# wsntxxn/AudioCaption

Measured on AMD Instinct MI355X. Metric: clips/sec (10 s @ 32 kHz) encode+greedy-decode, Cnn14_Rnn-Trm, higher is better.
Workload: dtype bf16x3

## Files before the change

### audiocaption_amd/_lib.py

```python
import ctypes
import os

import torch

_HERE = os.path.dirname(os.path.abspath(__file__))
LIB_PATH = os.environ.get("AUDIOCAPTION_HIP_LIB") or os.path.join(_HERE, "libaudiocaption_hip.so")

AC_MAX_LAYERS = 8
AC_ENS_MAX = 8
ABI_VERSION = 2

c_float_p = ctypes.c_void_p
c_int_p = ctypes.c_void_p


class AcTrmLayer(ctypes.Structure):
    _fields_ = [(n, ctypes.c_void_p) for n in (
        "sa_in_w", "sa_in_b", "sa_out_w", "sa_out_b", "ca_in_w", "ca_in_b", "ca_out_w", "ca_out_b",
        "l1_w", "l1_b", "l2_w", "l2_b", "n1_w", "n1_b", "n2_w", "n2_b", "n3_w", "n3_b")]


class AcTrmWeights(ctypes.Structure):
    _fields_ = [(n, ctypes.c_int32) for n in (
        "d_model", "nhead", "nlayers", "dim_ff", "vocab", "max_pos", "attn_emb_dim", "reserved")] + [
        (n, ctypes.c_void_p) for n in ("emb", "pe", "cls_w", "proj_w", "proj_b", "proj_ln_w", "proj_ln_b", "step_pk")] + [
        ("layer", AcTrmLayer * AC_MAX_LAYERS)]


class AcTrmKeyword(ctypes.Structure):
    _fields_ = [("kwp", ctypes.c_void_p), ("ln_w", ctypes.c_void_p), ("ln_b", ctypes.c_void_p), ("row_div", ctypes.c_int32)]


class AcLogitRules(ctypes.Structure):
    _fields_ = [("repetition_penalty", ctypes.c_float), ("no_repeat_ngram", ctypes.c_int32), ("min_length", ctypes.c_int32),
                ("end_idx", ctypes.c_int32), ("n_bad", ctypes.c_int32), ("bad_words", ctypes.c_void_p)]


class AcBahWeights(ctypes.Structure):
    _fields_ = [(n, ctypes.c_int32) for n in (
        "emb_dim", "d_model", "attn_size", "attn_emb_dim", "fc_emb_dim", "vocab", "n_tags", "variant")] + [
        (n, ctypes.c_void_p) for n in ("emb", "temb", "w_ih", "w_hh", "b_ih", "b_hh", "attn_w", "attn_b", "attn_v",
                                       "fc_w", "fc_b", "ctx_w", "ctx_b", "cls_w", "cls_b")]


class AcBahGrads(ctypes.Structure):
    _fields_ = [(n, ctypes.c_void_p) for n in ("emb", "temb", "w_ih", "w_hh", "b_ih", "b_hh", "attn_w", "attn_b", "attn_v",
                                               "fc_w", "fc_b", "ctx_w", "ctx_b", "cls_w", "cls_b")]


_I, _L, _F, _P = ctypes.c_int, ctypes.c_long, ctypes.c_float, ctypes.c_void_p
_U64 = ctypes.c_ulonglong
_WP = ctypes.POINTER(AcTrmWeights)
_BP = ctypes.c_void_p

SIGNATURES = {
    "ac_abi_version": (_I, []),
    "ac_logmel": (_I, [_P, _I, _I, _I, _I, _P, _P, _P, _P, _P, _P, _P, _P, _I, _L, _L, _L, _P]),
    "ac_conv3x3_bn_relu": (_I, [_P, _P, _P, _P, _P, _I, _I, _I, _I, _I, _I, _I, _I, _P]),
    "ac_conv3x3_bn_relu_winograd": (_I, [_P, _P, _P, _P, _P, _I, _I, _I, _I, _I, _I, _I, _I, _P]),
    "ac_conv3x3_bn_relu_bf16x3": (_I, [_P, _P, _P, _P, _P, _I, _I, _I, _I, _I, _I, _I, _I, _P]),
    "ac_conv3x3_bn_relu_bf16x3_gw": (_I, [_P, _P, _P, _P, _P, _I, _I, _I, _I, _I, _I, _I, _I, _P]),
    "ac_conv3x3_bn_relu_wino1d": (_I, [_P, _P, _P, _P, _P, _I, _I, _I, _I, _I, _I, _I, _I, _P, _I, _I, _P]),
    "ac_conv3x3_bn_relu_wino1d_drop": (_I, [_P, _P, _P, _P, _P, _I, _I, _I, _I, _I, _I, _I, _I, _F, _U64, _P, _P]),
    "ac_conv3x3_wino1d_splitk_floats": (_L, [_I, _I, _I, _I, _I]),
    "ac_conv3x3_bn_relu_wino1d_splitk": (_I, [_P, _P, _P, _P, _P, _I, _I, _I, _I, _I, _I, _I, _I, _P, _I, _I, _P, _L, _P]),
    "ac_conv3x3_bn_relu_wino43": (_I, [_P, _P, _P, _P, _P, _I, _I, _I, _I, _I, _I, _I, _I, _I, _P, _I, _I, _P]),
    "ac_conv3x3_bn_relu_wino43_drop": (_I, [_P, _P, _P, _P, _P, _I, _I, _I, _I, _I, _I, _I, _I, _F, _U64, _P, _P]),
    "ac_conv3x3_wino43_workgroups": (_L, [_I, _I, _I, _I]),
    "ac_conv3x3_block1_wino43": (_I, [_P, _P, _P, _P, _P, _P, _P, _P, _I, _I, _I, _P, _I, _I, _F, _U64, _P, _P]),
    "ac_conv3x3_block1_wino43_mfma": (_I, [_P, _P, _P, _P, _P, _P, _P, _P, _I, _I, _I, _P, _I, _I, _F, _U64, _P, _P]),
    "ac_conv3x3_block1_conv2_wino43": (_I, [_P, _P, _P, _P, _P, _I, _I, _I, _P]),
    "ac_conv3x3_bn_relu_f16x2_gw": (_I, [_P, _P, _P, _P, _P, _I, _I, _I, _I, _I, _I, _I, _I, _I, _P, _P]),
    "ac_conv3x3_block1_f16x2": (_I, [_P, _P, _P, _P, _P, _P, _P, _P, _I, _I, _I, _I, _P, _P]),
    "ac_linear_bf16x3": (_I, [_P, _P, _P, _P, _P, _I, _I, _I, _I, _P]),
    "ac_conv3x3_first": (_I, [_P, _P, _P, _P, _P, _I, _I, _I, _I, _P]),
    "ac_conv3x3_first_f16": (_I, [_P, _P, _P, _P, _P, _I, _I, _I, _I, _P, _P]),
    "ac_linear": (_I, [_P, _P, _P, _P, _I, _I, _I, _L, _L, _L, _I, _P]),
    "ac_gru_pack_whh": (_I, [_P, _P, _I, _P]),
    "ac_gru_layer": (_I, [_P, _P, _P, _P, _P, _I, _I, _I, _P]),
    "ac_gru_split_workspace_bytes": (_L, [_I]),
    "ac_gru_layer_split": (_I, [_P, _P, _P, _P, _P, _P, _P, _I, _I, _I, _P]),
    "ac_mean_with_lens": (_I, [_P, _P, _P, _I, _I, _I, _I, _P]),
    "ac_add_layernorm": (_I, [_P, _P, _P, _P, _P, _I, _I, _L, _L, _L, _P]),
    "ac_trm_memory": (_I, [_WP, _P, _I, _I, _P, _P, _P]),
    "ac_trm_step_pack_floats": (_L, [_WP]),
    "ac_trm_pack_step_weights": (_I, [_WP, _P, _P]),
    "ac_dec_wide_packed_floats": (_L, [_I, _I]),
    "ac_dec_wide_pack": (_I, [_P, _L, _I, _I, _P, _P]),
    "ac_dec_wide_gemm": (_I, [_I, _P, _L, _P, _L, _P, _P, _P, _L, _I, _P, _P, _F, _P, _L, _P, _P, _P, _L, _I, _I, _I, _I, _I, _I, _P]),
    "ac_trm_workspace_floats": (_L, [_WP, _I, _I]),
    "ac_trm_greedy": (_I, [_WP, _P, _P, _I, _I, _I, _I, _I, _I, _P, _P, _P, _P, _P, _P, _P]),
    "ac_trm_greedy_segments": (_I, [_WP, _P, _P, _I, _I, _I, _I, _I, _I, _I, _P, _P, _P, _P, _P, _P, _P]),
    "ac_sample_rows": (_I, [_P, _L, _I, _I, _I, _I, _F, _F, _P, _I, _P, _P, _P]),
    "ac_trm_sample": (_I, [_WP, _P, _P, _I, _I, _I, _I, _I, _I, _P, _P, _P, _P, _P, _P, _I, _I, _F, _F, _P, _P]),
    "ac_trm_sample_multi": (_I, [_WP, _P, _P, _I, _I, _I, _I, _I, _I, _I, _P, _P, _P, _P, _P, _P, _I, _I, _F, _F, _P, _P]),
    "ac_conv3x3_skinny_workspace_floats": (_L, [_I, _I, _I, _I, _I]),
    "ac_conv3x3_bn_relu_skinny": (_I, [_P, _P, _P, _P, _P, _I, _I, _I, _I, _I, _I, _I, _P, _L, _F, _U64, _P, _P]),
    "ac_trm_cluster_pack_floats": (_L, [_WP]),
    "ac_trm_cluster_pack": (_I, [_WP, _P, _P]),
    "ac_trm_cluster_workspace_bytes": (_L, [_I]),
    "ac_trm_greedy_cluster": (_I, [_WP, _P, _P, _P, _I, _I, _I, _I, _I, _I, _P, _P, _P, _P, _P, _P, _I, _P]),
    "ac_trm_forward_tokens": (_I, [_WP, _P, _P, _I, _I, _P, _P, _I, _P, _P, _P, _P]),
    "ac_trm_beam_step": (_I, [_WP, _P, _P, _I, _I, _I, _I, _I, _F, _P, _P, _P, _P, _P, _P, _P]),
    "ac_trm_beam_update": (_I, [_P, _P, _P, _P, _P, _P, _P, _P, _P, _P, _P, _P, _I, _I, _I, _I, _I, _I, _I, _I, _P]),
    "ac_trm_beam_reorder": (_I, [_WP, _I, _I, _I, _P, _P, _P]),
    "ac_trm_beam_update_all": (_I, [_P, _P, _P, _P, _P, _P, _P, _P, _P, _P, _P, _P, _I, _I, _I, _I, _I, _I, _I, _I, _P]),
    "ac_trm_kw_greedy_segments": (_I, [_WP, _P, _P, _P, _I, _I, _I, _I, _I, _I, _I, _P, _P, _P, _P, _P, _P, _P]),
    "ac_trm_kw_sample": (_I, [_WP, _P, _P, _P, _I, _I, _I, _I, _I, _I, _P, _P, _P, _P, _P, _P, _I, _I, _F, _F, _P, _P]),
    "ac_trm_kw_forward_tokens": (_I, [_WP, _P, _P, _P, _I, _I, _P, _P, _I, _P, _P, _P, _P]),
    "ac_trm_kw_beam_step": (_I, [_WP, _P, _P, _P, _I, _I, _I, _I, _I, _F, _P, _P, _P, _P, _P, _P, _P]),
    "ac_trm_kw_embed_qkv": (_I, [_WP, _P, _I, _I, _I, _P, _L, _P, _P, _P]),
    "ac_trm_step_logits": (_I, [_WP, _P, _P, _I, _I, _I, _I, _I, _P, _P, _I, _P, _L, _P, _L, _P, _P]),
    "ac_ens_greedy_pick": (_I, [_P, _I, _L, _I, _I, _I, _I, _I, _I, _P, _P, _P, _P, _P, _P, _P]),
    "ac_ens_sample_pick": (_I, [_P, _I, _L, _I, _I, _I, _I, _F, _F, _P, _I, _I, _I, _I, _P, _P, _P, _P, _P, _P, _P, _P]),
    "ac_ens_beam_step_select": (_I, [_P, _I, _L, _I, _I, _I, _I, _F, _P, _P, _P, _P, _P]),
    "ac_logit_rules_apply": (_I, [_P, _L, _P, _L, _I, _I, _P, _L, _I, _P, _P]),
    "ac_trm_search_rules": (_I, [_WP, _P, _P, _I, _I, _I, _I, _I, _I, _I, _P, _P, _P, _P, _P, _P, _I, _I, _F, _F, _P, _P, _P, _L,
                                 _P]),
    "ac_trm_beam_step_rules": (_I, [_WP, _P, _P, _I, _I, _I, _I, _I, _F, _P, _P, _P, _P, _P, _P, _P, _P, _P]),
    "ac_bah_workspace_floats": (_L, [_BP, _I, _I, _I, _I]),
    "ac_bah_memory": (_I, [_BP, _P, _P, _I, _I, _I, _I, _P, _P]),
    "ac_bah_memory_cond": (_I, [_BP, _P, _P, _I, _I, _I, _I, _P, _P]),
    "ac_bah_step_logits": (_I, [_BP, _P, _P, _I, _I, _I, _I, _I, _P, _P, _L, _P, _P, _P, _L, _P, _L, _P, _L, _L, _P, _P]),
    "ac_bah_greedy": (_I, [_BP, _P, _P, _P, _I, _I, _I, _I, _I, _I, _P, _P, _P, _P, _P, _P, _P, _P, _P]),
    "ac_bah_sample": (_I, [_BP, _P, _P, _P, _I, _I, _I, _I, _I, _I, _P, _P, _P, _P, _P, _P, _P, _P, _I, _I, _F, _F, _P, _P]),
    "ac_bah_beam_gather": (_I, [_P, _P, _P, _P, _P, _P, _P, _I, _I, _I, _I, _I, _I, _P]),
    "ac_bah_train_workspace_floats": (_L, [_BP, _I, _I, _I]),
    "ac_bah_train_forward": (_I, [_BP, _P, _P, _P, _P, _L, _P, _P, _I, _I, _I, _I, _F, _U64, _P, _P, _P, _P, _P, _P, _P, _P,
                                  _P]),
    "ac_bah_train_rollout": (_I, [_BP, _P, _P, _P, _P, _I, _I, _I, _I, _I, _F, _P, _P, _L, _F, _U64, _P, _P, _P, _P, _P, _P, _P,
                                  _P, _P, _P]),
    "ac_bah_train_backward": (_I, [_BP, _P, _P, _P, _P, _P, _I, _I, _I, _F, _U64, _P, _P, _P, _P, _P]),
    "ac_bah_train_forward_cond": (_I, [_BP, _P, _P, _P, _P, _L, _P, _I, _I, _I, _I, _F, _U64, _P, _P, _P, _P, _P, _P, _P, _P,
                                       _P]),
# ... 162 lines not shown
```

### audiocaption_amd/build.py

```python
import hashlib
import os
import shutil
import subprocess
import sys

HERE = os.path.dirname(os.path.abspath(__file__))
CSRC = os.path.join(HERE, "csrc")
LIB = os.path.join(HERE, "libaudiocaption_hip.so")
STAMP = LIB + ".stamp"
SOURCES = ["logmel.hip", "conv3x3.hip", "conv3x3_winograd.hip", "conv3x3_wino1d.hip", "conv3x3_wino43.hip", "conv3x3_block1_w4.hip", "conv3x3_skinny.hip", "gemm.hip", "gru.hip", "decoder.hip", "decoder_wide.hip", "decoder_cluster.hip", "sample.hip", "ensemble.hip", "logit_rules.hip", "attn_gru.hip", "attn_gru_train.hip", "spec_loss.hip", "sed.hip", "train.hip", "scst.hip", "kd.hip", "enc_kd.hip", "cider.hip", "capmetrics.hip", "diversity.hip", "effnet.hip", "effnet_fused.hip", "pw_gemm.hip", "ingest.hip", "probe.hip"]
FLAGS = ["--offload-arch=gfx950", "-O3", "-std=c++17", "-fPIC", "-Wall",
         "-Wno-unused-function", "-Wno-unused-result"]
NO_PACKED_F32 = ["-Xclang", "-target-feature", "-Xclang", "-packed-fp32-ops"]
EXTRA_FLAGS = {"sed.hip": ["-ffp-contract=off"], "enc_kd.hip": ["-ffp-contract=off"]}

def _hipcc():
    for c in (os.environ.get("HIPCC"), "/opt/rocm/bin/hipcc", shutil.which("hipcc")):
        if c and os.path.exists(c):
            return c
    raise RuntimeError("hipcc not found (expected /opt/rocm/bin/hipcc)")


def _digest():
    h = hashlib.sha256()
    for root in (CSRC, os.path.join(os.path.dirname(HERE), "include")):
        for name in sorted(os.listdir(root)):
            with open(os.path.join(root, name), "rb") as f:
                h.update(name.encode())
                h.update(f.read())
    h.update(" ".join(FLAGS).encode())
    h.update(repr((NO_PACKED_F32, sorted(EXTRA_FLAGS.items()))).encode())
    return h.hexdigest()


def _up_to_date(digest):
    if os.path.exists(LIB) and os.path.exists(STAMP):
        with open(STAMP) as f:
            return f.read().strip() == digest
    return False


def build(force=False, verbose=False):
    import fcntl
    digest = _digest()
    if not force and _up_to_date(digest):
        return LIB
    os.makedirs(os.path.join(HERE, "build"), exist_ok=True)
    with open(os.path.join(HERE, "build", ".lock"), "w") as lock:
        fcntl.flock(lock, fcntl.LOCK_EX)
        try:
            if not force and _up_to_date(digest):
                return LIB
            return _compile(digest, verbose)
        finally:
            fcntl.flock(lock, fcntl.LOCK_UN)


def _compile(digest, verbose):
    hipcc = _hipcc()
    objs = []
    procs = []
    os.makedirs(os.path.join(HERE, "build"), exist_ok=True)
    for src in SOURCES:
# ... 26 lines not shown
```

### audiocaption_amd/csrc/gru.hip

```cpp
#include "ac_common.h"

namespace {

struct GruParams {
  const float* gx;
  const float* whhT;
  const float* bhh;
  const int* lens;
  float* out;
  int B, T;
};

constexpr int H = 256;

__device__ __forceinline__ float sigmoidf_(float x) { return 1.0f / (1.0f + expf(-x)); }

constexpr int GRU_KREG = 96, GRU_KLDS = 48;
__global__ __launch_bounds__(768) void gru_layer_kernel(GruParams p) {
  __shared__ __attribute__((aligned(16))) float sh[H];
  __shared__ float sg[3 * H];
  extern __shared__ __attribute__((aligned(16))) float swl[];
  const int n = threadIdx.x;
  const int b = blockIdx.x >> 1, dir = blockIdx.x & 1;
  int len = p.lens[b];
// ... 171 lines not shown
  if (c >= C) return;
  const int len = lens[b];
  float s = 0.f;
  for (int t = 0; t < len && t < T; ++t) s += x[((size_t)b * T + t) * C + c];
  out[(size_t)b * C + c] = s / (float)len;
}

__global__ void maxmean_lens_kernel(const float* x, const int* lens, float* out, int T, int C) {
  const int b = blockIdx.x, c = blockIdx.y * blockDim.x + threadIdx.x;
  if (c >= C) return;
  const int len = lens[b];
  float s = 0.f, m = -INFINITY;
  for (int t = 0; t < len && t < T; ++t) {
    const float v = x[((size_t)b * T + t) * C + c];
    s += v;
    m = fmaxf(m, v);
  }
  out[(size_t)b * C + c] = m + s / (float)len;
}

__global__ void gru_pack_whh_kernel(const float* whh, float* packed, int total) {
  const int i = blockIdx.x * blockDim.x + threadIdx.x;
  if (i >= total) return;
  const int kk = i & 3, n = (i >> 2) % (3 * H), k4 = ((i >> 2) / (3 * H)) % (H / 4), d = i / (3 * H * H);
  packed[i] = whh[((size_t)d * 3 * H + n) * H + k4 * 4 + kk];
}

}

extern "C" int ac_gru_pack_whh(const float* whh, float* packed, int hidden, void* stream) {
  if (!whh || !packed || hidden != H) return AC_ERR_ARG;
  const int total = 2 * 3 * H * H;
  hipLaunchKernelGGL(gru_pack_whh_kernel, dim3((total + 255) / 256), dim3(256), 0, (hipStream_t)stream, whh, packed, total);
  return ac_check_launch();
}

extern "C" int ac_gru_layer(const float* gx, const float* whhT, const float* bhh, const int* lens, float* out,
                            int B, int T, int hidden, void* stream) {
  if (!gx || !whhT || !bhh || !lens || !out || B <= 0 || T <= 0 || hidden != H) return AC_ERR_ARG;
  GruParams p;
  p.gx = gx; p.whhT = whhT; p.bhh = bhh; p.lens = lens; p.out = out; p.B = B; p.T = T;
  const size_t lds = (size_t)GRU_KLDS * 3 * H * sizeof(float);
  static AcLdsAttr lds_attr;
  if (ac_allow_lds((const void*)gru_layer_kernel, (int)lds, &lds_attr) != AC_OK) return AC_ERR_LAUNCH;
  hipLaunchKernelGGL(gru_layer_kernel, dim3(2 * B), dim3(768), lds, (hipStream_t)stream, p);
  return ac_check_launch();
}

extern "C" long ac_gru_split_workspace_bytes(int B) {
  if (B <= 0) return AC_ERR_ARG;
  return 128 + (long)B * 2 * GQ * 2 * HQ * 8;
}

extern "C" int ac_gru_layer_split(const float* gx, const float* whh, const float* bhh, const int* lens, float* out,
                                  float* save, void* workspace, int B, int T, int hidden, void* stream) {
  if (!gx || !whh || !bhh || !lens || !out || !workspace || B <= 0 || T <= 0 || hidden != H) return AC_ERR_ARG;
  const size_t gran = (size_t)B * 2 * GQ * 2 * HQ * 8;
  GruSplitParams p;
  p.gx = gx; p.whh = whh; p.bhh = bhh; p.lens = lens; p.out = out; p.save = save; p.B = B; p.T = T;
  p.error = (unsigned*)workspace;
  p.ticket = (unsigned*)((char*)workspace + 64);
  p.xch = (unsigned long long*)((char*)workspace + 128);
  {
    const unsigned words = (unsigned)((64 + gran) / 8);
    hipLaunchKernelGGL(gru_split_reset_kernel, dim3((words + 255) / 256), dim3(256), 0, (hipStream_t)stream,
                       (unsigned long long*)((char*)workspace + 64), words);
  }
  hipLaunchKernelGGL(gru_layer_split_kernel, dim3(2 * GQ * B), dim3(256), 0, (hipStream_t)stream, p);
  return ac_check_launch();
}

extern "C" int ac_mean_with_lens(const float* x, const int* lens, float* out, int B, int T, int C, int add_max,
                                 void* stream) {
  if (!x || !lens || !out || B <= 0 || T <= 0 || C <= 0) return AC_ERR_ARG;
  if (add_max)
    hipLaunchKernelGGL(maxmean_lens_kernel, dim3(B, (C + 255) / 256), dim3(256), 0, (hipStream_t)stream, x, lens, out, T, C);
  else
    hipLaunchKernelGGL(mean_lens_kernel, dim3(B, (C + 255) / 256), dim3(256), 0, (hipStream_t)stream, x, lens, out, T, C);
  return ac_check_launch();
}
```

### audiocaption_amd/kernels.py

```python
import contextlib
import ctypes
import os

import torch

from . import _lib
from ._lib import check, f32c, ptr, stream


def upload(t, device, dtype=None):
    t = torch.as_tensor(t)
    if t.is_cuda:
        return t.to(device=device, dtype=dtype)
    if dtype is not None:
        t = t.to(dtype)
    pin = torch.empty(t.shape, dtype=t.dtype, pin_memory=True)
    pin.copy_(t)
    return pin.to(device, non_blocking=True)


def _dev(t):
    if not t.is_cuda:
        raise _lib.HipLibraryError("the HIP path needs tensors on a ROCm device; there is no CPU fallback")
    return t
# ... 261 lines not shown

    return torch.stack([lay(hi), lay(lo)], dim=3).contiguous()


def pack_conv_weight_winograd(w):
    cout, cin = w.shape[0], w.shape[1]

    def g_times(t, dim):
        t0, t1, t2 = t.select(dim, 0), t.select(dim, 1), t.select(dim, 2)
        return torch.stack([t0, 0.5 * (t0 + t1 + t2), 0.5 * (t0 - t1 + t2), t2], dim=dim)

    out = torch.empty(cin // 32, 4, 4, cout, 32, device=w.device, dtype=torch.float32)
    step = max(1, (1 << 22) // (cin * 16))
    for o0 in range(0, cout, step):
        u = g_times(g_times(w[o0:o0 + step].double(), 2), 3)
        u = u.permute(1, 3, 2, 0).reshape(cin // 32, 32, 4, 4, -1).permute(0, 2, 3, 4, 1)
        out[:, :, :, o0:o0 + step] = u.float()
    return out


def pack_conv_weight(w):
    cout, cin = w.shape[0], w.shape[1]
    return (w.permute(1, 2, 3, 0).reshape(cin // 32, 32, 9, cout).permute(0, 2, 3, 1).contiguous())


def fold_bn(bn_weight, bn_bias, mean, var, eps):
    scale = bn_weight / torch.sqrt(var + eps)
    return scale.contiguous(), (bn_bias - mean * scale).contiguous()


LINEAR_ALGO = os.environ.get("AUDIOCAPTION_LINEAR_ALGO", "bf16x3")
_LINEAR_PACKS = {}


def pack_linear_weight_bf16x3_frag(w):
    n, k = w.shape
    return pack_conv_weight_bf16x3_frag(w.reshape(n, k, 1, 1))


def _linear_pack(w):
    import weakref
    hit = _LINEAR_PACKS.get(id(w))
    if hit is not None and hit[0]() is w and hit[1] == w._version and hit[2] == _lib.param_generation():
        return hit[3:]
    for k in [k for k, v in _LINEAR_PACKS.items() if v[0]() is None]:
        del _LINEAR_PACKS[k]
    with torch.no_grad():
        pack = (pack_linear_weight_bf16x3_frag(w.detach().float()), torch.ones(w.shape[0], device=w.device),
                torch.zeros(w.shape[0], device=w.device))
    _LINEAR_PACKS[id(w)] = (weakref.ref(w), w._version, _lib.param_generation()) + pack
    return pack


def linear(x, w, b=None, relu=False, out=None):
    lib = _lib.load()
    M, K = x.shape
    N = w.shape[0]
    if out is None:
        out = torch.empty(M, N, device=x.device, dtype=torch.float32)
    if (LINEAR_ALGO == "bf16x3" and N * K >= 1536 * 512 and K % 32 == 0 and N % 64 == 0 and x.stride(0) == K
            and out.stride(0) == N and w.is_contiguous()):
        wfrag, ones, zeros = _linear_pack(w)
        check(lib.ac_linear_bf16x3(ptr(x), ptr(wfrag), ptr(ones), ptr(b if b is not None else zeros), ptr(out), M, N, K,
                                   1 if relu else 0, stream()), "ac_linear_bf16x3")
        return out
    check(lib.ac_linear(ptr(x), ptr(w), ptr(b), ptr(out), M, N, K, x.stride(0), w.stride(0), out.stride(0),
                        1 if relu else 0, stream()), "ac_linear")
    return out


def gru_pack_whh(whh, hidden):
    lib = _lib.load()
    whh = f32c(_dev(whh))
    out = torch.empty_like(whh)
    check(lib.ac_gru_pack_whh(ptr(whh), ptr(out), hidden, stream()), "ac_gru_pack_whh")
    return out


def gru_layer(gx, whhT, bhh, lens_i32, B, T, hidden):
    lib = _lib.load()
    out = torch.empty(B, T, 2 * hidden, device=gx.device, dtype=torch.float32)
    check(lib.ac_gru_layer(ptr(gx), ptr(whhT), ptr(bhh), ptr(lens_i32), ptr(out), B, T, hidden, stream()),
          "ac_gru_layer")
    return out


def gru_layer_split(gx, whh, bhh, lens_i32, B, T, hidden, workspace=None):
    lib = _lib.load()
    need = lib.ac_gru_split_workspace_bytes(B)
    if workspace is None or workspace.numel() * 8 < need or workspace.device != gx.device:
        workspace = torch.zeros((need + 7) // 8, device=gx.device, dtype=torch.int64)
    out = torch.empty(B, T, 2 * hidden, device=gx.device, dtype=torch.float32)
    check(lib.ac_gru_layer_split(ptr(gx), ptr(whh), ptr(bhh), ptr(lens_i32), ptr(out), None, ptr(workspace), B, T, hidden,
                                 stream()), "ac_gru_layer_split")
    return out, workspace


def gru_split_error(workspace, B):
    return workspace.view(torch.int32)[:1]


def mean_with_lens(x, lens_i32, add_max=False):
    lib = _lib.load()
    B, T, C = x.shape
    out = torch.empty(B, C, device=x.device, dtype=torch.float32)
    check(lib.ac_mean_with_lens(ptr(x), ptr(lens_i32), ptr(out), B, T, C, 1 if add_max else 0, stream()),
          "ac_mean_with_lens")
    return out


def add_layernorm(x, y, w, b, out=None):
    lib = _lib.load()
    rows, d = x.shape
    if out is None:
        out = torch.empty(rows, d, device=x.device, dtype=torch.float32)
    check(lib.ac_add_layernorm(ptr(x), ptr(y), ptr(w), ptr(b), ptr(out), rows, d, x.stride(0),
                               y.stride(0) if y is not None else 0, out.stride(0), stream()), "ac_add_layernorm")
    return out


def dropout_(x, n, p, seed, seed_dev=None):
    lib = _lib.load()
    check(lib.ac_dropout(ptr(x), ptr(x), n, float(p), int(seed), seed_dev, 0, stream()), "ac_dropout")
    return x


def rows_mean_w(x, out, B, Hp, H, W, C):
    lib = _lib.load()
    check(lib.ac_rows_mean_w(ptr(x), ptr(out), B, Hp, H, W, C, stream()), "ac_rows_mean_w")
    return out


def specaug_(x, stripes, fill, B, rows_per_clip, T, n_time=2, n_freq=2):
    lib = _lib.load()
    check(lib.ac_specaug(ptr(x), ptr(stripes), ptr(fill), B, rows_per_clip, T, 64, n_time, n_freq, stream()), "ac_specaug")
    return x


def specaug_stripes(seed, B, T, F=64, time_width=64, time_num=2, freq_width=8, freq_num=2):
    import numpy as np
    rng = np.random.default_rng(int(seed) & 0xFFFFFFFFFFFFFFFF)
    out = np.zeros((B, time_num + freq_num, 2), dtype=np.int32)
    for b in range(B):
        for k in range(time_num):
            d = int(rng.integers(0, time_width))
            out[b, k] = (int(rng.integers(0, T - d)), d)
    for b in range(B):
# ... 43 lines not shown
```

### audiocaption_amd/rnn_encoder.py

```python
import os

import torch
import torch.nn as nn

from . import kernels as K


class RnnEncoder(nn.Module):

    def __init__(self, spec_dim, fc_feat_dim, attn_feat_dim, pooling="mean", **kwargs):
        super().__init__()
        self.spec_dim, self.fc_feat_dim, self.attn_feat_dim = spec_dim, fc_feat_dim, attn_feat_dim
        self.pooling = pooling
        self.hidden_size = kwargs.get("hidden_size", 512)
        self.bidirectional = kwargs.get("bidirectional", False)
        self.num_layers = kwargs.get("num_layers", 1)
        self.dropout = kwargs.get("dropout", 0.2)
        self.rnn_type = kwargs.get("rnn_type", "GRU")
        self.in_bn = kwargs.get("in_bn", False)
        self.embed_dim = self.hidden_size * (self.bidirectional + 1)
        if self.rnn_type != "GRU" or not self.bidirectional or self.hidden_size != 256 or self.in_bn:
            raise NotImplementedError(
                "RnnEncoder (HIP path) is built for the configuration the reference configs use: "
                "rnn_type=GRU, bidirectional=True, hidden_size=256, in_bn=False "
                "(eg_configs/*/waveform/cnn14rnn_trm.yaml:18-27)")
        if self.pooling != "mean":
            raise NotImplementedError("RnnEncoder (HIP path): only pooling='mean' is built")
        self.network = nn.GRU(attn_feat_dim, self.hidden_size, num_layers=self.num_layers,
                              bidirectional=True, dropout=self.dropout, batch_first=True)
        self._packed = None
        self._packed_key = None
        self.gru_algo = os.environ.get("AUDIOCAPTION_GRU_ALGO", "split")
        self._split_ws = None

    def _pack(self):
        ps = dict(self.network.named_parameters())
        key = tuple((t.data_ptr(), t._version) for t in ps.values()) + (K._lib.param_generation(),)
        if self._packed is not None and key == self._packed_key:
            return self._packed
        layers = []
        with torch.no_grad():
            for l in range(self.num_layers):
                f, r = f"_l{l}", f"_l{l}_reverse"
                w_ih = torch.cat([ps["weight_ih" + f], ps["weight_ih" + r]], 0).float().contiguous()
                b_ih = torch.cat([ps["bias_ih" + f], ps["bias_ih" + r]], 0).float().contiguous()
                whh = torch.stack([ps["weight_hh" + f], ps["weight_hh" + r]], 0).float().contiguous()
                whhT = K.gru_pack_whh(whh, self.hidden_size)
                bhh = torch.stack([ps["bias_hh" + f], ps["bias_hh" + r]], 0).float().contiguous()
                layers.append((w_ih, b_ih, whhT, bhh, whh))
        self._packed, self._packed_key = layers, key
        return layers

    def forward(self, input_dict):
        if self.training:
            raise NotImplementedError(
                "RnnEncoder (HIP path): in train mode the GRU only runs inside the whole-model training step "
                "(audiocaption_amd.train.TrainEngine / TransformerModel.forward with mode='train')")
        x = input_dict["attn"]
        lens = torch.as_tensor(input_dict["attn_len"]).cpu().long()
        B, T, _ = x.shape
        if int(lens.min()) < 1 or int(lens.max()) > T:
            raise ValueError("attn_len must lie in [1, attn.size(1)]")
        lens_dev = K.upload(lens, x.device, torch.int32)
        h = K.f32c(x).reshape(B * T, -1)
        algo = input_dict.get("gru_algo", self.gru_algo)
        split = algo == "split"
        for (w_ih, b_ih, whhT, bhh, whh) in self._pack():
            gx = K.linear(h, w_ih, b_ih)
            if split:
                h, self._split_ws = K.gru_layer_split(gx, whh, bhh, lens_dev, B, T, self.hidden_size, self._split_ws)
                h = h.reshape(B * T, -1)
            else:
                h = K.gru_layer(gx, whhT, bhh, lens_dev, B, T, self.hidden_size).reshape(B * T, -1)
        out = h.reshape(B, T, self.embed_dim)
        t_out = int(lens.max())
        if t_out < T:
            out = out[:, :t_out].contiguous()
        fc_emb = K.mean_with_lens(out, lens_dev)
        res = {"attn_emb": out, "fc_emb": fc_emb, "attn_emb_len": lens}
        if split:
            res["gru_error"] = K.gru_split_error(self._split_ws, B)
        return res
```

### include/audiocaption_hip.h

```cpp
#ifndef AUDIOCAPTION_HIP_H
#define AUDIOCAPTION_HIP_H

#include <stdint.h>

#ifdef __cplusplus
extern "C" {
#endif

#define AC_OK 0
#define AC_ERR_ARG (-1)
#define AC_ERR_LAUNCH (-2)

#define AC_ABI_VERSION 2
int ac_abi_version(void);

int ac_logmel(const float* wav, int B, int L, int n_fft, int hop, const float* window, const float* twiddle,
              const float* melfb, const int* mel_lo, const int* mel_hi, const float* scale, const float* shift,
              float* out, int rows_per_clip, long stride_b, long stride_t, long stride_m, void* stream);

int ac_conv3x3_bn_relu(const float* in, const float* wpk, const float* scale, const float* shift, float* out,
                       int B, int Hp, int H, int W, int Cin, int Cout, int mode, int map_mode, void* stream);
int ac_conv3x3_bn_relu_winograd(const float* in, const float* upk, const float* scale, const float* shift,
                                float* out, int B, int Hp, int H, int W, int Cin, int Cout, int mode,
                                int map_mode, void* stream);
int ac_conv3x3_bn_relu_bf16x3(const float* in, const void* wpk, const float* scale, const float* shift, float* out,
                              int B, int Hp, int H, int W, int Cin, int Cout, int mode, int map_mode, void* stream);
int ac_conv3x3_bn_relu_bf16x3_gw(const float* in, const void* wfrag, const float* scale, const float* shift,
                                 float* out, int B, int Hp, int H, int W, int Cin, int Cout, int mode,
                                 int map_mode, void* stream);
int ac_conv3x3_bn_relu_wino1d(const float* in, const void* wfrag, const float* scale, const float* shift,
                              float* out, int B, int Hp, int H, int W, int Cin, int Cout, int mode,
                              int map_mode, const int* clip_frames, int need_mul, int need_add, void* stream);
int ac_conv3x3_bn_relu_wino1d_drop(const float* in, const void* wfrag, const float* scale, const float* shift,
                                   float* out, int B, int Hp, int H, int W, int Cin, int Cout, int mode, int map_mode,
                                   float drop_p, unsigned long long drop_seed, const unsigned long long* seed_dev,
                                   void* stream);
long ac_conv3x3_wino1d_splitk_floats(int B, int Hp, int W, int Cin, int Cout);
int ac_conv3x3_bn_relu_wino1d_splitk(const float* in, const void* wfrag, const float* scale, const float* shift,
                                     float* out, int B, int Hp, int H, int W, int Cin, int Cout, int mode,
                                     int map_mode, const int* clip_frames, int need_mul, int need_add,
                                     float* workspace, long workspace_floats, void* stream);

long ac_conv3x3_skinny_workspace_floats(int B, int Hp, int W, int Cin, int Cout);
int ac_conv3x3_bn_relu_skinny(const float* in, const void* wfrag, const float* scale, const float* shift, float* out, int B,
                              int Hp, int H, int W, int Cin, int Cout, int mode, float* workspace, long workspace_floats,
                              float drop_p, unsigned long long drop_seed, const unsigned long long* seed_dev, void* stream);

int ac_conv3x3_bn_relu_wino43(const float* in, const void* wfrag, const float* scale, const float* shift, float* out,
                              int B, int Hp, int H, int W, int Cin, int Cout, int mode, int map_mode, int tiles_per_wave,
                              const int* clip_frames, int need_mul, int need_add, void* stream);
int ac_conv3x3_bn_relu_wino43_drop(const float* in, const void* wfrag, const float* scale, const float* shift, float* out,
                                   int B, int Hp, int H, int W, int Cin, int Cout, int mode, int map_mode, float drop_p,
                                   unsigned long long drop_seed, const unsigned long long* seed_dev, void* stream);
long ac_conv3x3_wino43_workgroups(int B, int Hp, int W, int Cout);

int ac_conv3x3_block1_wino43(const float* in1, const float* w1, const float* scale1, const float* shift1,
                             const void* wfrag2, const float* scale2, const float* shift2, float* out, int B, int Hp,
                             int H, const int* clip_frames, int need_mul, int need_add, float drop_p,
                             unsigned long long drop_seed, const unsigned long long* seed_dev, void* stream);
int ac_conv3x3_block1_wino43_mfma(const float* in1, const float* w1, const float* scale1, const float* shift1,
                                  const void* wfrag2, const float* scale2, const float* shift2, float* out, int B, int Hp,
                                  int H, const int* clip_frames, int need_mul, int need_add, float drop_p,
                                  unsigned long long drop_seed, const unsigned long long* seed_dev, void* stream);
int ac_conv3x3_block1_conv2_wino43(const float* in64, const void* wfrag2, const float* scale2, const float* shift2,
                                   float* out, int B, int Hp, int H, void* stream);

int ac_conv3x3_bn_relu_f16x2_gw(const void* in, const void* wfrag, const float* scale, const float* shift,
                                void* out, int B, int Hp, int H, int W, int Cin, int Cout, int mode,
                                int map_mode, int out_f32, unsigned int* overflow_flag, void* stream);
int ac_conv3x3_block1_f16x2(const float* in1, const float* w1, const float* scale1, const float* shift1,
                            const void* wfrag2, const float* scale2, const float* shift2, void* out,
                            int B, int Hp, int H, int W, unsigned int* overflow_flag, void* stream);

int ac_linear_bf16x3(const float* X, const void* wfrag, const float* ones, const float* bias, float* Y,
                     int M, int N, int K, int relu, void* stream);

int ac_conv3x3_first(const float* in, const float* w, const float* scale, const float* shift, float* out,
                     int B, int Hp, int H, int W, void* stream);
int ac_conv3x3_first_f16(const float* in, const float* w, const float* scale, const float* shift, void* out,
                         int B, int Hp, int H, int W, unsigned int* overflow_flag, void* stream);

int ac_linear(const float* X, const float* W, const float* bias, float* Y, int M, int N, int K, long ldx,
              long ldw, long ldy, int relu, void* stream);

int ac_gru_pack_whh(const float* whh, float* packed, int hidden, void* stream);
int ac_gru_layer(const float* gx, const float* whhT, const float* bhh, const int* lens, float* out, int B,
                 int T, int hidden, void* stream);
long ac_gru_split_workspace_bytes(int B);
int ac_gru_layer_split(const float* gx, const float* whh, const float* bhh, const int* lens, float* out, float* save,
                       void* workspace, int B, int T, int hidden, void* stream);
int ac_mean_with_lens(const float* x, const int* lens, float* out, int B, int T, int C, int add_max,
                      void* stream);

#define AC_MAX_LAYERS 8
typedef struct {
  const float *sa_in_w, *sa_in_b, *sa_out_w, *sa_out_b;
  const float *ca_in_w, *ca_in_b, *ca_out_w, *ca_out_b;
  const float *l1_w, *l1_b, *l2_w, *l2_b;
  const float *n1_w, *n1_b, *n2_w, *n2_b, *n3_w, *n3_b;
} ac_trm_layer;

typedef struct {
  int32_t d_model, nhead, nlayers, dim_ff, vocab, max_pos, attn_emb_dim, reserved;
  const float* emb;
  const float* pe;
  const float* cls_w;
  const float* proj_w;
  const float* proj_b;
  const float* proj_ln_w;
  const float* proj_ln_b;
  const float* step_pk;
  ac_trm_layer layer[AC_MAX_LAYERS];
} ac_trm_weights;

int ac_add_layernorm(const float* x, const float* y, const float* w, const float* b, float* out, int rows,
                     int d, long ldx, long ldy, long ldo, void* stream);

int ac_trm_memory(const ac_trm_weights* w, const float* attn_emb, int R, int Tm, float* memkv, float* tmp,
                  void* stream);

long ac_trm_step_pack_floats(const ac_trm_weights* w);
int ac_trm_pack_step_weights(const ac_trm_weights* w, float* out, void* stream);

long ac_dec_wide_packed_floats(int N, int K);
int ac_dec_wide_pack(const float* W, long ldw, int N, int K, float* out, void* stream);
int ac_dec_wide_gemm(int producer, const float* X, long ldx, const float* Y2, long ldy2, const float* ln_w,
                     const float* ln_b, const int* tok, long tok_stride, int t, const float* emb, const float* pe,
                     float emb_scale, float* xout, long ldxo, const float* Wp, const float* bias, float* Y, long ldy, int M,
                     int N, int K, int relu, int ntb, int split_out, void* stream);

long ac_trm_workspace_floats(const ac_trm_weights* w, int rows, int max_len);

int ac_trm_greedy(const ac_trm_weights* w, const float* memkv, const int* mem_len, int B, int Tm, int max_len,
                  int start_idx, int end_idx, int pad_idx, int64_t* seq, float* logit, float* logprob,
                  float* embed, int* unfinished_cnt, float* ws, void* stream);

int ac_trm_greedy_segments(const ac_trm_weights* w, const float* memkv, const int* mem_len, int B, int segments, int Tm,
                           int max_len, int start_idx, int end_idx, int pad_idx, int64_t* seq, float* logit,
                           float* logprob, float* embed, int* unfinished_cnt, float* ws, void* stream);

long ac_trm_cluster_pack_floats(const ac_trm_weights* w);
int ac_trm_cluster_pack(const ac_trm_weights* w, float* out, void* stream);
long ac_trm_cluster_workspace_bytes(int B);
// ... 341 lines not shown
```

Measured before the change: 15790.

## Add LDS-tiled split-bf16 linear kernel and fold GRU workspace reset into it

Adds a new 128x128x64 LDS-tiled bf16x3 GEMM kernel for large linear layers. It double-buffers hi/lo splits of the activations in LDS, prefetches weight fragments into registers, and makes tiled the default route. The GRU input projection kernel also zeroes the split-GRU workspace, so the separate reset kernel launch can be skipped through a new prezeroed entry point. The cost is extra LDS, a launch-bounds occupancy of 1, and a correctness dependency: the GRU must only run prezeroed when the preceding linear actually took the tiled route.

```diff
diff --git a/audiocaption_amd/_lib.py b/audiocaption_amd/_lib.py
--- a/audiocaption_amd/_lib.py
+++ b/audiocaption_amd/_lib.py
@@ -73,6 +73,9 @@
     "ac_conv3x3_bn_relu_f16x2_gw": (_I, [_P, _P, _P, _P, _P, _I, _I, _I, _I, _I, _I, _I, _I, _I, _P, _P]),
     "ac_conv3x3_block1_f16x2": (_I, [_P, _P, _P, _P, _P, _P, _P, _P, _I, _I, _I, _I, _P, _P]),
     "ac_linear_bf16x3": (_I, [_P, _P, _P, _P, _P, _I, _I, _I, _I, _P]),
+    "ac_linear_tiled_pack_bytes": (_L, [_I, _I]),
+    "ac_linear_tiled_workgroups": (_L, [_I, _I, _I]),
+    "ac_linear_bf16x3_tiled": (_I, [_P, _P, _P, _P, _I, _I, _I, _I, _P, _L, _P]),
     "ac_conv3x3_first": (_I, [_P, _P, _P, _P, _P, _I, _I, _I, _I, _P]),
     "ac_conv3x3_first_f16": (_I, [_P, _P, _P, _P, _P, _I, _I, _I, _I, _P, _P]),
     "ac_linear": (_I, [_P, _P, _P, _P, _I, _I, _I, _L, _L, _L, _I, _P]),
@@ -80,6 +83,7 @@
     "ac_gru_layer": (_I, [_P, _P, _P, _P, _P, _I, _I, _I, _P]),
     "ac_gru_split_workspace_bytes": (_L, [_I]),
     "ac_gru_layer_split": (_I, [_P, _P, _P, _P, _P, _P, _P, _I, _I, _I, _P]),
+    "ac_gru_layer_split_prezeroed": (_I, [_P, _P, _P, _P, _P, _P, _P, _I, _I, _I, _P]),
     "ac_mean_with_lens": (_I, [_P, _P, _P, _I, _I, _I, _I, _P]),
     "ac_add_layernorm": (_I, [_P, _P, _P, _P, _P, _I, _I, _L, _L, _L, _P]),
     "ac_trm_memory": (_I, [_WP, _P, _I, _I, _P, _P, _P]),
diff --git a/audiocaption_amd/build.py b/audiocaption_amd/build.py
--- a/audiocaption_amd/build.py
+++ b/audiocaption_amd/build.py
@@ -8,7 +8,7 @@
 CSRC = os.path.join(HERE, "csrc")
 LIB = os.path.join(HERE, "libaudiocaption_hip.so")
 STAMP = LIB + ".stamp"
-SOURCES = ["logmel.hip", "conv3x3.hip", "conv3x3_winograd.hip", "conv3x3_wino1d.hip", "conv3x3_wino43.hip", "conv3x3_block1_w4.hip", "conv3x3_skinny.hip", "gemm.hip", "gru.hip", "decoder.hip", "decoder_wide.hip", "decoder_cluster.hip", "sample.hip", "ensemble.hip", "logit_rules.hip", "attn_gru.hip", "attn_gru_train.hip", "spec_loss.hip", "sed.hip", "train.hip", "scst.hip", "kd.hip", "enc_kd.hip", "cider.hip", "capmetrics.hip", "diversity.hip", "effnet.hip", "effnet_fused.hip", "pw_gemm.hip", "ingest.hip", "probe.hip"]
+SOURCES = ["logmel.hip", "conv3x3.hip", "conv3x3_winograd.hip", "conv3x3_wino1d.hip", "conv3x3_wino43.hip", "conv3x3_block1_w4.hip", "conv3x3_skinny.hip", "linear_bf16x3.hip", "gemm.hip", "gru.hip", "decoder.hip", "decoder_wide.hip", "decoder_cluster.hip", "sample.hip", "ensemble.hip", "logit_rules.hip", "attn_gru.hip", "attn_gru_train.hip", "spec_loss.hip", "sed.hip", "train.hip", "scst.hip", "kd.hip", "enc_kd.hip", "cider.hip", "capmetrics.hip", "diversity.hip", "effnet.hip", "effnet_fused.hip", "pw_gemm.hip", "ingest.hip", "probe.hip"]
 FLAGS = ["--offload-arch=gfx950", "-O3", "-std=c++17", "-fPIC", "-Wall",
          "-Wno-unused-function", "-Wno-unused-result"]
 NO_PACKED_F32 = ["-Xclang", "-target-feature", "-Xclang", "-packed-fp32-ops"]
diff --git a/audiocaption_amd/csrc/ac_linear_tiled.h b/audiocaption_amd/csrc/ac_linear_tiled.h
--- /dev/null
+++ b/audiocaption_amd/csrc/ac_linear_tiled.h
@@ -0,0 +1,46 @@
+#pragma once
+#include <stddef.h>
+#include <stdint.h>
+
+#ifndef AC_OK
+#define AC_OK 0
+#define AC_ERR_ARG (-1)
+#define AC_ERR_LAUNCH (-2)
+#endif
+
+enum {
+  LT_BM = 128,
+  LT_BN = 128,
+  LT_BK = 64,
+  LT_PITCH = LT_BK + 8,
+  LT_OPITCH = 72,
+};
+
+struct LinTiledPlan {
+  unsigned grid;
+  int row_tiles, col_tiles;
+  size_t lds_bytes;
+};
+
+static inline long ac_linear_tiled_pack_bytes_(int N, int K) {
+  if (N <= 0 || K <= 0 || N % LT_BN || K % LT_BK) return AC_ERR_ARG;
+  return (long)N * K * 2 * 2;
+}
+
+static inline int ac_linear_tiled_plan(const void* X, const void* wfrag, const void* bias, const void* Y, int M, int N, int K,
+                                       const void* zero_ws, long zero_bytes, LinTiledPlan* plan) {
+  if (!X || !wfrag || !bias || !Y || !plan) return AC_ERR_ARG;
+  if (M <= 0 || N <= 0 || K <= 0 || N % LT_BN || K % LT_BK) return AC_ERR_ARG;
+  if (((uintptr_t)X | (uintptr_t)wfrag | (uintptr_t)bias | (uintptr_t)Y) & 15u) return AC_ERR_ARG;
+  if (zero_bytes < 0 || (zero_bytes && !zero_ws) || (zero_bytes & 7) || ((uintptr_t)zero_ws & 7u)) return AC_ERR_ARG;
+  if (zero_bytes / 8 > 0x7fffffffL) return AC_ERR_ARG;
+  const long long rt = ((long long)M + LT_BM - 1) / LT_BM, ct = N / LT_BN;
+  if (rt * ct > (1LL << 22)) return AC_ERR_ARG;
+  plan->row_tiles = (int)rt;
+  plan->col_tiles = (int)ct;
+  plan->grid = (unsigned)(rt * ct);
+  const size_t a_bytes = (size_t)2 * 2 * LT_BM * LT_PITCH * 2;
+  const size_t o_bytes = (size_t)4 * 64 * LT_OPITCH * 4;
+  plan->lds_bytes = a_bytes > o_bytes ? a_bytes : o_bytes;
+  return AC_OK;
+}
diff --git a/audiocaption_amd/csrc/gru.hip b/audiocaption_amd/csrc/gru.hip
--- a/audiocaption_amd/csrc/gru.hip
+++ b/audiocaption_amd/csrc/gru.hip
@@ -247,8 +247,8 @@
   return 128 + (long)B * 2 * GQ * 2 * HQ * 8;
 }
 
-extern "C" int ac_gru_layer_split(const float* gx, const float* whh, const float* bhh, const int* lens, float* out,
-                                  float* save, void* workspace, int B, int T, int hidden, void* stream) {
+static int gru_layer_split_launch(const float* gx, const float* whh, const float* bhh, const int* lens, float* out,
+                                  float* save, void* workspace, int B, int T, int hidden, void* stream, bool reset) {
   if (!gx || !whh || !bhh || !lens || !out || !workspace || B <= 0 || T <= 0 || hidden != H) return AC_ERR_ARG;
   const size_t gran = (size_t)B * 2 * GQ * 2 * HQ * 8;
   GruSplitParams p;
@@ -256,13 +256,23 @@
   p.error = (unsigned*)workspace;
   p.ticket = (unsigned*)((char*)workspace + 64);
   p.xch = (unsigned long long*)((char*)workspace + 128);
-  {
+  if (reset) {
     const unsigned words = (unsigned)((64 + gran) / 8);
     hipLaunchKernelGGL(gru_split_reset_kernel, dim3((words + 255) / 256), dim3(256), 0, (hipStream_t)stream,
                        (unsigned long long*)((char*)workspace + 64), words);
   }
   hipLaunchKernelGGL(gru_layer_split_kernel, dim3(2 * GQ * B), dim3(256), 0, (hipStream_t)stream, p);
   return ac_check_launch();
+}
+
+extern "C" int ac_gru_layer_split(const float* gx, const float* whh, const float* bhh, const int* lens, float* out,
+                                  float* save, void* workspace, int B, int T, int hidden, void* stream) {
+  return gru_layer_split_launch(gx, whh, bhh, lens, out, save, workspace, B, T, hidden, stream, true);
+}
+
+extern "C" int ac_gru_layer_split_prezeroed(const float* gx, const float* whh, const float* bhh, const int* lens, float* out,
+                                            float* save, void* workspace, int B, int T, int hidden, void* stream) {
+  return gru_layer_split_launch(gx, whh, bhh, lens, out, save, workspace, B, T, hidden, stream, false);
 }
 
 extern "C" int ac_mean_with_lens(const float* x, const int* lens, float* out, int B, int T, int C, int add_max,
diff --git a/audiocaption_amd/csrc/linear_bf16x3.hip b/audiocaption_amd/csrc/linear_bf16x3.hip
--- /dev/null
+++ b/audiocaption_amd/csrc/linear_bf16x3.hip
@@ -0,0 +1,179 @@
+#include "ac_wino43.h"
+#include "ac_linear_tiled.h"
+
+namespace {
+
+struct LinTiledParams {
+  const float* x;
+  const bf16x8* w;
+  const float* bias;
+  float* y;
+  int M, N, K, row_tiles;
+  unsigned long long* zero;
+  unsigned zero_words;
+};
+
+constexpr int LT_PLANE = LT_BM * LT_PITCH;
+
+template <bool RELU>
+__global__ __launch_bounds__(256, 1) void linear_bf16x3_tiled_kernel(LinTiledParams p) {
+  extern __shared__ __attribute__((aligned(16))) unsigned char lt_smem[];
+  const int tid = threadIdx.x, lane = tid & 63, wave = tid >> 6;
+  const int wm = wave >> 1, wn = wave & 1, half = lane >> 5;
+  const int m_tile = (int)(blockIdx.x % (unsigned)p.row_tiles), n_tile = (int)(blockIdx.x / (unsigned)p.row_tiles);
+  const int m0 = m_tile * LT_BM, n0 = n_tile * LT_BN;
+
+  for (unsigned i = blockIdx.x * 256u + tid; i < p.zero_words; i += gridDim.x * 256u) p.zero[i] = 0ull;
+
+  __bf16* sA = (__bf16*)lt_smem;
+
+  const int r0 = tid >> 4, c4 = tid & 15;
+  const float* xrow[8];
+#pragma unroll
+  for (int j = 0; j < 8; ++j) {
+    int g = m0 + r0 + 16 * j;
+    g = g < p.M ? g : p.M - 1;
+    xrow[j] = p.x + (size_t)g * p.K + c4 * 4;
+  }
+  const int soff = r0 * LT_PITCH + c4 * 4;
+  f32x4 pre[8];
+  auto request = [&](int c) {
+#pragma unroll
+    for (int j = 0; j < 8; ++j) pre[j] = *(const f32x4*)(xrow[j] + c * LT_BK);
+  };
+  auto commit = [&](int buf) {
+    __bf16* dh = sA + buf * 2 * LT_PLANE + soff;
+#pragma unroll
+    for (int j = 0; j < 8; ++j) {
+      u32x2 hi, lo;
+      split_bf16x4(pre[j], hi, lo);
+      *(u32x2*)(dh + j * 16 * LT_PITCH) = hi;
+      *(u32x2*)(dh + LT_PLANE + j * 16 * LT_PITCH) = lo;
+    }
+  };
+
+  const size_t kstride = (size_t)(p.N >> 5) * 128;
+  const bf16x8* wbase = p.w + (size_t)(n_tile * 4 + wn * 2) * 128 + lane;
+  bf16x8 w[4][2][2];
+  auto w_load = [&](int g, int slot) {
+#pragma unroll
+    for (int n = 0; n < 2; ++n)
+#pragma unroll
+      for (int pl = 0; pl < 2; ++pl) w[slot][n][pl] = wbase[(size_t)g * kstride + n * 128 + pl * 64];
+  };
+
+  f32x16 acc[2][2];
+#pragma unroll
+  for (int m = 0; m < 2; ++m)
+#pragma unroll
+    for (int n = 0; n < 2; ++n)
+#pragma unroll
+      for (int r = 0; r < 16; ++r) acc[m][n][r] = 0.f;
+
+  const int arow = (wm * 64 + (lane & 31)) * LT_PITCH + half * 8;
+  const int nchunk = p.K / LT_BK;
+  request(0);
+  __builtin_amdgcn_sched_barrier(0);
+#pragma unroll
+  for (int kk = 0; kk < 4; ++kk) {
+    w_load(kk, kk);
+    __builtin_amdgcn_sched_barrier(0);
+  }
+  commit(0);
+  lds_barrier();
+#pragma unroll 1
+  for (int c = 0; c < nchunk; ++c) {
+    const int cn = c + 1 < nchunk ? c + 1 : c;
+    request(cn);
+    __builtin_amdgcn_sched_barrier(0);
+    const __bf16* ahp = sA + (c & 1) * 2 * LT_PLANE + arow;
+    const __bf16* alp = ahp + LT_PLANE;
+    bf16x8 ah[2][2], al[2][2];
+    auto frags = [&](int kk) {
+#pragma unroll
+      for (int m = 0; m < 2; ++m) {
+        ah[kk & 1][m] = *(const bf16x8*)(ahp + m * 32 * LT_PITCH + kk * 16);
+        al[kk & 1][m] = *(const bf16x8*)(alp + m * 32 * LT_PITCH + kk * 16);
+      }
+    };
+    frags(0);
+#pragma unroll
+    for (int kk = 0; kk < 4; ++kk) {
+      if (kk < 3) frags(kk + 1);
+      else commit((c + 1) & 1);
+      const int f = kk & 1;
+#pragma unroll
+      for (int m = 0; m < 2; ++m)
+#pragma unroll
+        for (int n = 0; n < 2; ++n) acc[m][n] = __builtin_amdgcn_mfma_f32_32x32x16_bf16(al[f][m], w[kk][n][0], acc[m][n], 0, 0, 0);
+#pragma unroll
+      for (int m = 0; m < 2; ++m)
+#pragma unroll
+        for (int n = 0; n < 2; ++n) acc[m][n] = __builtin_amdgcn_mfma_f32_32x32x16_bf16(ah[f][m], w[kk][n][1], acc[m][n], 0, 0, 0);
+#pragma unroll
+      for (int m = 0; m < 2; ++m)
+#pragma unroll
+        for (int n = 0; n < 2; ++n) acc[m][n] = __builtin_amdgcn_mfma_f32_32x32x16_bf16(ah[f][m], w[kk][n][0], acc[m][n], 0, 0, 0);
+      w_load(cn * 4 + kk, kk);
+      __builtin_amdgcn_sched_barrier(0);
+    }
+    lds_barrier();
+  }
+
+  float* so = (float*)lt_smem + wave * 64 * LT_OPITCH;
+#pragma unroll
+  for (int m = 0; m < 2; ++m)
+#pragma unroll
+    for (int n = 0; n < 2; ++n)
+#pragma unroll
+      for (int r = 0; r < 16; ++r)
+        so[(m * 32 + (r & 3) + 8 * (r >> 2) + 4 * half) * LT_OPITCH + n * 32 + (lane & 31)] = acc[m][n][r];
+  const int ocol = (lane & 15) * 4;
+  const int gcol = n0 + wn * 64 + ocol;
+  const f32x4 b4 = *(const f32x4*)(p.bias + gcol);
+#pragma unroll
+  for (int it = 0; it < 16; ++it) {
+    const int row = it * 4 + (lane >> 4);
+    const int grow = m0 + wm * 64 + row;
+    f32x4 v = *(const f32x4*)(so + row * LT_OPITCH + ocol);
+#pragma unroll
+    for (int e = 0; e < 4; ++e) {
+      v[e] = v[e] + b4[e];
+      if (RELU) v[e] = fmaxf(v[e], 0.f);
+    }
+    if (grow < p.M) *(f32x4*)(p.y + (size_t)grow * p.N + gcol) = v;
+  }
+}
+
+template <bool RELU>
+int launch_linear_tiled(const LinTiledParams& p, const LinTiledPlan& plan, hipStream_t s) {
+  static AcLdsAttr lds_attr;
+  if (ac_allow_lds((const void*)linear_bf16x3_tiled_kernel<RELU>, (int)plan.lds_bytes, &lds_attr) != AC_OK) return AC_ERR_LAUNCH;
+  hipLaunchKernelGGL((linear_bf16x3_tiled_kernel<RELU>), dim3(plan.grid), dim3(256), plan.lds_bytes, s, p);
+  return ac_check_launch();
+}
+
+}
+
+extern "C" long ac_linear_tiled_pack_bytes(int N, int K) { return ac_linear_tiled_pack_bytes_(N, K); }
+
+extern "C" long ac_linear_tiled_workgroups(int M, int N, int K) {
+  LinTiledPlan plan;
+  alignas(16) static const char aligned = 0;
+  const int rc = ac_linear_tiled_plan(&aligned, &aligned, &aligned, &aligned, M, N, K, nullptr, 0, &plan);
+  return rc == AC_OK ? (long)plan.grid : (long)rc;
+}
+
+extern "C" int ac_linear_bf16x3_tiled(const float* X, const void* wfrag, const float* bias, float* Y, int M, int N, int K,
+                                      int relu, void* zero_ws, long zero_bytes, void* stream) {
+  LinTiledPlan plan;
+  const int rc = ac_linear_tiled_plan(X, wfrag, bias, Y, M, N, K, zero_ws, zero_bytes, &plan);
+  if (rc != AC_OK) return rc;
+  LinTiledParams p;
+  p.x = X; p.w = (const bf16x8*)wfrag; p.bias = bias; p.y = Y;
+  p.M = M; p.N = N; p.K = K; p.row_tiles = plan.row_tiles;
+  p.zero = (unsigned long long*)zero_ws;
+  p.zero_words = (unsigned)(zero_bytes / 8);
+  hipStream_t s = (hipStream_t)stream;
+  return relu ? launch_linear_tiled<true>(p, plan, s) : launch_linear_tiled<false>(p, plan, s);
+}
diff --git a/audiocaption_amd/kernels.py b/audiocaption_amd/kernels.py
--- a/audiocaption_amd/kernels.py
+++ b/audiocaption_amd/kernels.py
@@ -337,16 +337,39 @@
     return pack
 
 
-def linear(x, w, b=None, relu=False, out=None):
+LINEAR_KERNEL = os.environ.get("AUDIOCAPTION_LINEAR_KERNEL", "tiled")
+
+
+def linear_route(x, w, b=None, out=None):
+    M, K = x.shape
+    N = w.shape[0]
+    if not (LINEAR_ALGO == "bf16x3" and N * K >= 1536 * 512 and K % 32 == 0 and N % 64 == 0 and x.stride(0) == K
+            and (out is None or out.stride(0) == N) and w.is_contiguous()):
+        return "f32"
+    if LINEAR_KERNEL not in ("tiled", "onetap"):
+        raise ValueError(f"AUDIOCAPTION_LINEAR_KERNEL={LINEAR_KERNEL!r}: 'tiled' or 'onetap'")
+    aligned = all(t is None or t.data_ptr() % 16 == 0 for t in (x, b, out))
+    return "tiled" if LINEAR_KERNEL == "tiled" and N % 128 == 0 and K % 64 == 0 and aligned else "onetap"
+
+
+def linear(x, w, b=None, relu=False, out=None, zero_ws=None):
     lib = _lib.load()
     M, K = x.shape
     N = w.shape[0]
     if out is None:
         out = torch.empty(M, N, device=x.device, dtype=torch.float32)
-    if (LINEAR_ALGO == "bf16x3" and N * K >= 1536 * 512 and K % 32 == 0 and N % 64 == 0 and x.stride(0) == K
-            and out.stride(0) == N and w.is_contiguous()):
+    route = linear_route(x, w, b, out)
+    if zero_ws is not None and route != "tiled":
+        raise ValueError("linear: zero_ws needs the tiled split-bf16 route (linear_route)")
+    if route != "f32":
         wfrag, ones, zeros = _linear_pack(w)
-        check(lib.ac_linear_bf16x3(ptr(x), ptr(wfrag), ptr(ones), ptr(b if b is not None else zeros), ptr(out), M, N, K,
+        bias = b if b is not None else zeros
+        if route == "tiled":
+            zp, zn = (zero_ws[0].data_ptr() + zero_ws[1], zero_ws[2]) if zero_ws is not None else (None, 0)
+            check(lib.ac_linear_bf16x3_tiled(ptr(x), ptr(wfrag), ptr(bias), ptr(out), M, N, K, 1 if relu else 0, zp, zn,
+                                             stream()), "ac_linear_bf16x3_tiled")
+            return out
+        check(lib.ac_linear_bf16x3(ptr(x), ptr(wfrag), ptr(ones), ptr(bias), ptr(out), M, N, K,
                                    1 if relu else 0, stream()), "ac_linear_bf16x3")
         return out
     check(lib.ac_linear(ptr(x), ptr(w), ptr(b), ptr(out), M, N, K, x.stride(0), w.stride(0), out.stride(0),
@@ -370,14 +393,27 @@
     return out
 
 
-def gru_layer_split(gx, whh, bhh, lens_i32, B, T, hidden, workspace=None):
-    lib = _lib.load()
-    need = lib.ac_gru_split_workspace_bytes(B)
-    if workspace is None or workspace.numel() * 8 < need or workspace.device != gx.device:
-        workspace = torch.zeros((need + 7) // 8, device=gx.device, dtype=torch.int64)
+def gru_split_workspace(B, device, workspace=None):
+    need = _lib.load().ac_gru_split_workspace_bytes(B)
+    if workspace is None or workspace.numel() * 8 < need or workspace.device != device:
+        workspace = torch.zeros((need + 7) // 8, device=device, dtype=torch.int64)
+    return workspace
+
+
+def gru_split_zero_region(workspace, B):
+    return workspace, 64, _lib.load().ac_gru_split_workspace_bytes(B) - 64
+
+
+def gru_layer_split(gx, whh, bhh, lens_i32, B, T, hidden, workspace=None, prezeroed=False):
+    lib = _lib.load()
+    ws = gru_split_workspace(B, gx.device, workspace)
+    if prezeroed and ws is not workspace:
+        raise ValueError("gru_layer_split: prezeroed needs the workspace that was zeroed")
+    workspace = ws
     out = torch.empty(B, T, 2 * hidden, device=gx.device, dtype=torch.float32)
-    check(lib.ac_gru_layer_split(ptr(gx), ptr(whh), ptr(bhh), ptr(lens_i32), ptr(out), None, ptr(workspace), B, T, hidden,
-                                 stream()), "ac_gru_layer_split")
+    fn = lib.ac_gru_layer_split_prezeroed if prezeroed else lib.ac_gru_layer_split
+    check(fn(ptr(gx), ptr(whh), ptr(bhh), ptr(lens_i32), ptr(out), None, ptr(workspace), B, T, hidden, stream()),
+          "ac_gru_layer_split")
     return out, workspace
 
 
diff --git a/audiocaption_amd/rnn_encoder.py b/audiocaption_amd/rnn_encoder.py
--- a/audiocaption_amd/rnn_encoder.py
+++ b/audiocaption_amd/rnn_encoder.py
@@ -65,10 +65,15 @@
         h = K.f32c(x).reshape(B * T, -1)
         algo = input_dict.get("gru_algo", self.gru_algo)
         split = algo == "split"
+        if split:
+            self._split_ws = K.gru_split_workspace(B, x.device, self._split_ws)
         for (w_ih, b_ih, whhT, bhh, whh) in self._pack():
-            gx = K.linear(h, w_ih, b_ih)
+            fold = split and K.linear_route(h, w_ih, b_ih) == "tiled"
+            gx = K.linear(h, w_ih, b_ih,
+                          zero_ws=K.gru_split_zero_region(self._split_ws, B) if fold else None)
             if split:
-                h, self._split_ws = K.gru_layer_split(gx, whh, bhh, lens_dev, B, T, self.hidden_size, self._split_ws)
+                h, self._split_ws = K.gru_layer_split(gx, whh, bhh, lens_dev, B, T, self.hidden_size, self._split_ws,
+                                                      prezeroed=fold)
                 h = h.reshape(B * T, -1)
             else:
                 h = K.gru_layer(gx, whhT, bhh, lens_dev, B, T, self.hidden_size).reshape(B * T, -1)
diff --git a/include/audiocaption_hip.h b/include/audiocaption_hip.h
--- a/include/audiocaption_hip.h
+++ b/include/audiocaption_hip.h
@@ -74,6 +74,10 @@
 
 int ac_linear_bf16x3(const float* X, const void* wfrag, const float* ones, const float* bias, float* Y,
                      int M, int N, int K, int relu, void* stream);
+long ac_linear_tiled_pack_bytes(int N, int K);
+long ac_linear_tiled_workgroups(int M, int N, int K);
+int ac_linear_bf16x3_tiled(const float* X, const void* wfrag, const float* bias, float* Y, int M, int N, int K, int relu,
+                           void* zero_ws, long zero_bytes, void* stream);
 
 int ac_conv3x3_first(const float* in, const float* w, const float* scale, const float* shift, float* out,
                      int B, int Hp, int H, int W, void* stream);
@@ -89,6 +93,8 @@
 long ac_gru_split_workspace_bytes(int B);
 int ac_gru_layer_split(const float* gx, const float* whh, const float* bhh, const int* lens, float* out, float* save,
                        void* workspace, int B, int T, int hidden, void* stream);
+int ac_gru_layer_split_prezeroed(const float* gx, const float* whh, const float* bhh, const int* lens, float* out,
+                                 float* save, void* workspace, int B, int T, int hidden, void* stream);
 int ac_mean_with_lens(const float* x, const int* lens, float* out, int B, int T, int C, int add_max,
                       void* stream);
 
```

Measured after the change: 15930, median of 6. No clear change (+0.9%).
